# kkaytekin/Supervised-Depth-Estimation-from-Polarized-Images

Measured on AMD Instinct MI355X. Metric: train images/sec (512x612, 3-encoder), higher is better.
Workload: dtype f32; 1 GPU; BASELINE configs[2]: full 3-encoder (augment_xolp+augment_normals), multi-scale loss scales=[0,1,2,3], batch 16 per GPU, 512x612 frames (network/loss on 512x640 padded), dropout 0.1, Adam lr 1e-4, fp32; global_batch=16, height=512, width=640, frame_width=612, parallelism=dp1

## Files before the change

include/polardepth.h:

```cpp
#ifndef POLARDEPTH_H
#define POLARDEPTH_H

#include <stddef.h>
#include <stdint.h>

#ifdef __cplusplus
extern "C" {
#endif

#define PD_OK 0
#define PD_EINVAL (-22)
#define PD_ELAUNCH (-5)

const char* pd_last_error(void);
int pd_version(void);

#define PD_POLAR_LS 0
#define PD_POLAR_STOKES 1
#define PD_POLAR_PRECISE_NORMALS 1
#define PD_POLAR_IEEE_RHO 2
#define PD_POLAR_NT_LOADS 4
#define PD_POLAR_PLAIN_LOADS 8

size_t pd_polar_tables_bytes(int n_d, int n_s1, int n_s2);
// ... 12 lines not shown

int pd_polar_calc_normals(const void* phi, const void* theta, void* out, int B, long P, int phi_f64, int theta_f64,
                          void* stream);

int pd_polar_theta(const void* rho, void* theta_d, void* theta_s1, void* theta_s2, void* bins,
                   const void* tables, size_t tables_bytes, long n, void* stream);

#define PD_CONV_AUTO 0u
#define PD_CONV_FP32_MFMA 1u
#define PD_CONV_BF16X3 2u
#define PD_CONV_WGRAD_SPLIT_IN_REGS 4u
#define PD_CONV_GENERAL_KERNELS 8u
#define PD_CONV_X3_IM2COL 16u
#define PD_CONV_WGRAD_ROW_WORKGROUPS 32u
#define PD_CONV_BF16 128u
#define PD_CONV_FLAGS_ALL 191u
int pd_conv2d_tile_m(long M, int Cout);
long pd_conv2d_stats_rows(long M, int Cout);
int pd_conv2d_uses_x3(long M, int Cout, int C, int KH, int KW, int stride, int pad, int mode, int act, int has_out_scale,
                      int Ho, int Wo, unsigned flags);
int pd_conv2d_uses_bf16(long M, int Cout, int C, int KH, int KW, int stride, int pad, int mode, int act, int has_out_scale,
                        int Ho, int Wo, unsigned flags);
int pd_conv2d(const void* x, const void* w, const void* bias, const void* out_scale, void* y, void* stats,
              int N, int H, int W, int C, long sN, long sH, long sW, long sC,
              int Ho, int Wo, int Cout, int KH, int KW, int stride, int pad, int mode, int act,
              int affine, float sub, float div, long ldy, unsigned flags, void* stream);

int pd_conv16(const void* x, const void* w, const void* bias, void* y, int N, int H, int W, int C,
              long sN, long sH, long sW, int Ho, int Wo, int Cout, long ldy, int mode, int act, void* stream);

size_t pd_conv16_wgrad_workspace(int C);
int pd_conv16_wgrad(const void* x, const void* dz, void* dw, void* dbias, void* workspace, size_t ws_bytes,
                    int N, int H, int W, int C, long sN, long sH, long sW, long ldd, int accumulate, void* stream);

int pd_dgrad_s2_filters(const void* wt, void* wsub, int Cin, int Cout, void* stream);
int pd_conv2d_rect(const void* x, const void* w, void* y, int N, int H, int W, int C, long sN, long sH, long sW, long sC,
                   int Ho, int Wo, int Cout, int KH, int KW, int pad_h, int pad_w, int mode, long ldy, unsigned flags,
                   void* stream);
int pd_interleave4(const void* sub, void* dx, int N, int Ho, int Wo, int C, void* stream);

int pd_conv2d_add(const void* x, const void* w, const void* addend, long ld_add, void* y,
                  int N, int H, int W, int C, long sN, long sH, long sW, long sC,
                  int Ho, int Wo, int Cout, int KH, int KW, int stride, int pad, int mode, long ldy, unsigned flags,
                  void* stream);

size_t pd_conv2d_wgrad_workspace(long M, int Cout, int K, unsigned flags);
int pd_conv2d_wgrad(const void* x, const void* dy, void* dw, void* dbias, void* workspace, size_t ws_bytes,
                    int N, int H, int W, int C, long sN, long sH, long sW, long sC,
                    int Ho, int Wo, int Cout, int KH, int KW, int stride, int pad, int mode,
                    int affine, float sub, float div, long ldd, int accumulate, unsigned flags, void* stream);
int pd_conv2d_wgrad_uses_x3(long M, int Cout, int C, int KH, int KW, int stride, int pad, int mode, int H, int W, int Ho, int Wo,
                            unsigned flags);
int pd_conv2d_wgrad_uses_bf16(long M, int Cout, int C, int KH, int KW, int stride, int pad, int mode, int H, int W, int Ho, int Wo,
                              unsigned flags);

int pd_stem_s2d_input(const void* x, void* out, int N, int C, int H, int W, long sN, long sC, long sH, long sW,
                      int affine, float sub, float div, void* stream);
int pd_stem_s2d_weight(const void* w, void* w2, int Cout, int C, void* stream);
int pd_stem_s2d_weight_grad(const void* dw2, void* dw, int Cout, int C, int accumulate, void* stream);
// ... 131 lines not shown
```

supervised-depth-estimation-from-polarized-images_amd/csrc/conv.hip:

```cpp
#include "pd_common.h"
#include <cstdlib>
#include <type_traits>

namespace {

typedef float f32x16 __attribute__((ext_vector_type(16)));
typedef unsigned int u32x4 __attribute__((ext_vector_type(4)));

constexpr int BK = 32;
constexpr int LDT = BK;
constexpr int NT = 256;
constexpr unsigned OOB = 0x80000000u;

enum { MODE_ZERO = 0, MODE_REFLECT = 1, MODE_TRANSPOSED = 2 };
enum { ACT_NONE = 0, ACT_RELU = 1, ACT_ELU = 2, ACT_SIGMOID = 3 };

struct ConvArgs {
    const float* x;
    const float* w;
    const float* bias;
    const float* oscale;
    float* y;
    float* stats;
    const float* add;
// ... 4 lines not shown
    int KH, KW, stride, pad;
    int pad_w;
    int mode, act;
    int affine;
    float sub, div;
    int K;
    long M;
    long ldy;
    int mtiles, ntiles;
    int sshift;
    unsigned w_bytes;
    unsigned mg_hw, sh_hw, mg_wo, sh_wo;
    unsigned flags;
    int stats_rows;
    int nmajor;
};

__device__ __forceinline__ float4 ldg4(const float* p) { return *reinterpret_cast<const float4*>(p); }

__device__ __forceinline__ int swz(int row, int slot) { return 4 * (slot ^ ((row >> 1) & 7)); }

__device__ __forceinline__ __amdgpu_buffer_rsrc_t make_rsrc(const void* p, unsigned bytes) {
    return __builtin_amdgcn_make_buffer_rsrc(const_cast<void*>(p), 0, bytes, 0x00020000);
}
__device__ __forceinline__ float4 buf_ld4(__amdgpu_buffer_rsrc_t r, unsigned off) {
    return __builtin_bit_cast(float4, __builtin_amdgcn_raw_buffer_load_b128(r, off, 0, 0));
}
__device__ __forceinline__ float buf_ld1(__amdgpu_buffer_rsrc_t r, unsigned off) {
    return __builtin_bit_cast(float, __builtin_amdgcn_raw_buffer_load_b32(r, off, 0, 0));
}
// ... 637 lines not shown
template <int P, bool W = false> __device__ __forceinline__ void sp_m(const float* x, Terms& t) {
    if constexpr (PD_PROBE_RAW(W)) { t.m[P] = __float_as_uint(x[2 * P + 1]); return; }
    t.tf[P] = f32x2{__uint_as_float(t.h[P] << 16), __uint_as_float(t.h[P] & 0xffff0000u)};
    t.tr[P] = f32x2{x[2 * P], x[2 * P + 1]} - t.tf[P];
    t.m[P] = cvt_pk_bf16(t.tr[P].x, t.tr[P].y);
    t.tf[P].x = __uint_as_float(t.m[P] << 16);
}
template <int P, bool W = false> __device__ __forceinline__ void sp_l(Terms& t) {
    if constexpr (PD_PROBE_RAW(W)) { t.l[P] = t.h[P]; return; }
    t.tf[P].y = __uint_as_float(t.m[P] & 0xffff0000u);
    const f32x2 r2 = t.tr[P] - t.tf[P];
    t.l[P] = cvt_pk_bf16(r2.x, r2.y);
}
}

template <int MODE, int RB = 2>
__global__ __launch_bounds__(NT, RB == 2 ? 3 : 4) void conv_igemm_x3_kernel(const ConvArgs a) {
    using namespace x3;
    constexpr int BM = 128 * RB;
    constexpr unsigned A_BYTES = BM * CK * 4, BS_BASE = 2 * A_BYTES, BP_BASE = BS_BASE + 2 * BS_BYTES;
    constexpr unsigned LDS_BYTES = BP_BASE + 2 * 3 * BP_BYTES;
    __shared__ __attribute__((aligned(16))) float smem_all[LDS_BYTES / 4];

    const int nblk = a.mtiles * a.ntiles;
    const int per_xcd = (int)gridDim.x >> 3;
    const int logical = ((int)blockIdx.x & 7) * per_xcd + ((int)blockIdx.x >> 3);
    if (logical >= nblk) return;
    const int mt = a.nmajor ? logical % a.mtiles : logical / a.ntiles, nt = a.nmajor ? logical / a.mtiles : logical - mt * a.ntiles;
    const long m0 = (long)mt * BM;
    const int n0 = nt * BN;

    const int tid = threadIdx.x;
    const int lane = tid & 63;
    const int wave = __builtin_amdgcn_readfirstlane(tid >> 6);
    const int hw = a.Ho * a.Wo;

    const unsigned wsign = (mt & 1) ? 0x80008000u : 0u;
    const int img0 = (int)(m0 / hw);
    const long shift = MODE != MODE_TRANSPOSED ? (long)a.pad * a.sH + (long)a.pad_w * a.sW
                                               : (long)(a.KH - 1 - a.pad) * a.sH + (long)(a.KW - 1 - a.pad_w) * a.sW;
    const long rest = (((long)a.N - img0) * a.sN + shift) * 4;
    const __amdgpu_buffer_rsrc_t rx = make_rsrc(a.x + (long)img0 * a.sN - shift, rest > 0x7fffffffL ? 0x7fffffffu : (unsigned)rest);
    const __amdgpu_buffer_rsrc_t rw_ = make_rsrc(a.w, a.w_bytes);
// ... 27 lines not shown
            hi_w = ow + a.pad_w + 1; lo_w = hi_w - a.W;
        }
        lo_h = min(max(lo_h, 0), a.KH); hi_h = min(max(hi_h, 0), a.KH);
        lo_w = min(max(lo_w, 0), a.KW); hi_w = min(max(hi_w, 0), a.KW);
        const unsigned bad_h = ((1u << lo_h) - 1u) | ~((1u << hi_h) - 1u);
        const unsigned bad_w = (((1u << lo_w) - 1u) | ~((1u << hi_w) - 1u)) & ones_kw;
        unsigned mask = 0;
        for (int kh = a.KH - 1; kh >= 0; --kh)
            mask = (mask << a.KW) | (((bad_h >> kh) & 1u) ? ones_kw : bad_w);
        inv[i] = m < a.M ? (mask | 0x80000000u) : 0xffffffffu;
    }
    const unsigned vb = (unsigned)((n0 + 16 * wave + prow) * a.K) * 4u + col4;

    const int dW4 = (MODE != MODE_TRANSPOSED ? (int)a.sW : -(int)a.sW) * 4, dH4 = (MODE != MODE_TRANSPOSED ? (int)a.sH : -(int)a.sH) * 4;
    const int ngroups = (a.C + CK - 1) / CK;
    const int nchunks = ngroups * a.KH * a.KW;
    const int c_lim = a.C - 4 * ((lane & 3) ^ ((lane >> 4) & 3));
    const int ntaps = a.KH * a.KW;
    const unsigned aoff0 = MODE != MODE_TRANSPOSED ? 0u : (unsigned)(((a.KH - 1) * (int)a.sH + (a.KW - 1) * (int)a.sW) * 4);
    int s_q = 0, s_tap = 0, s_kw = 0, s_kh = 0, s_c = 0;
    unsigned s_aoff = aoff0;
    int s_qb = 0, sb_tap = 0;
    unsigned s_boff = 0, sb_c4 = 0;
    const unsigned lds0 = (unsigned)(size_t)(lds_ptr_t*)smem_all;
    const unsigned m0_a = lds0 + 2048u * RB * (unsigned)wave, m0_b = lds0 + BS_BASE + 1024u * (unsigned)wave;

    auto load_a = [&](auto dst_tag, auto piece_tag) {
        constexpr unsigned DST = decltype(dst_tag)::value;
        constexpr int P = decltype(piece_tag)::value;
        if constexpr (MODE == MODE_REFLECT) {
            const int hs = s_kh == 0 ? max(hcor[P], 0) : s_kh == 2 ? min(hcor[P], 0) : 0;
            const int ws = s_kw == 0 ? max(wcor[P], 0) : s_kw == 2 ? min(wcor[P], 0) : 0;
            const unsigned bad = (s_tap == 31 ? 1u : 0u) | ((unsigned)(c_lim - 1 - s_c) >> 31);
            dma16s(rx, m0_a + DST * A_BYTES + 1024u * P, (bad << 31) + (va[P] + (unsigned)(hs + ws)), s_aoff);
        } else {
        const unsigned bad = __builtin_amdgcn_ubfe(inv[P], (unsigned)s_tap, 1u) | ((unsigned)(c_lim - 1 - s_c) >> 31);
        dma16s(rx, m0_a + DST * A_BYTES + 1024u * P, (bad << 31) + va[P], s_aoff);
        }
// ... 138 lines not shown
        const std::integral_constant<unsigned, 1> d1{};
        pieces<0, 2 * RB>(load_a, d0);
        advance_a();
        load_b(d0);
        load_b(d1);
        asm volatile("s_waitcnt vmcnt(0)" ::: "memory");
        __syncthreads();
        split_b(d0);
        __syncthreads();
    }
    for (int q = 0; q < nchunks; q += 2) {
        chunk(std::integral_constant<unsigned, 0>{});
        if (q + 1 < nchunks) chunk(std::integral_constant<unsigned, 1>{});
    }

    {
        constexpr int RW = 32 * RB;
        float* T = smem_all + wave * (RW * 32);
        float (*red)[BN][2] = reinterpret_cast<float (*)[BN][2]>(smem_all + 4 * RW * 32);
        const int col_l = lane & 31, rbase = 4 * (lane >> 5);
        const bool elu = a.act == ACT_ELU;
        const long rows_here = a.M - m0 < BM ? a.M - m0 : BM;
        const __amdgpu_buffer_rsrc_t ry = make_rsrc(a.y + m0 * a.ldy, (unsigned)(rows_here * a.ldy * 4));
        const __amdgpu_buffer_rsrc_t ra = make_rsrc(a.add ? a.add + m0 * a.ld_add : a.y, a.add ? (unsigned)(rows_here * a.ld_add * 4) : 0u);
#pragma unroll
        for (int j = 0; j < 2; ++j) {
            float4 addv[4 * RB];
            if (a.add) {
                const unsigned off_a = (unsigned)((RW * wave + (lane >> 3)) * (int)a.ld_add + n0 + 32 * j + 4 * (lane & 7)) * 4u;
#pragma unroll
// ... 63 lines not shown
           (!a.add || ((a.ld_add & 3) == 0 && ((size_t)a.add & 15) == 0)) && (long)a.Co * a.K * 4 < 0x7fffffffL;
}
static int x3_eligible(const ConvArgs& a, bool vec) {
    const bool force = (a.flags & PD_CONV_BF16X3) != 0;
    if (!(x3_common_ok(a, vec) && (a.C + x3::CK - 1) / x3::CK * x3::CK <= 2 * a.C && a.Co % x3::BN == 0 &&
          (a.M % 128 == 0 || (a.mode == MODE_TRANSPOSED && !a.stats))))
        return 0;
    const long ct = a.Co / x3::BN;
    if (a.M % 256 == 0 && (a.M / 256) * ct >= X3_MIN_WG) return 2;
    return (force || (a.M / 128) * ct >= X3_MIN_WG1) ? 1 : 0;
}

static int x3_nmajor(const ConvArgs& a) { return (long)a.Co * a.K * 4 > (3L << 20) && a.ntiles >= 8 && a.ntiles % 8 == 0; }
#include "conv_x3_halo.hpp"

static int launch_conv_x3(ConvArgs& a, int rb, hipStream_t st) {
    a.mtiles = (int)((a.M + 128 * rb - 1) / (128 * rb));
    a.ntiles = a.Co / x3::BN;
    a.nmajor = x3_nmajor(a);
    const long nblk = (long)a.mtiles * a.ntiles;
    const dim3 grid((unsigned)((nblk + 7) / 8 * 8)), block(NT);
    if (rb == 2) {
        if (a.mode == MODE_ZERO) hipLaunchKernelGGL((conv_igemm_x3_kernel<MODE_ZERO, 2>), grid, block, 0, st, a);
        else if (a.mode == MODE_REFLECT) hipLaunchKernelGGL((conv_igemm_x3_kernel<MODE_REFLECT, 2>), grid, block, 0, st, a);
        else hipLaunchKernelGGL((conv_igemm_x3_kernel<MODE_TRANSPOSED, 2>), grid, block, 0, st, a);
    } else {
        if (a.mode == MODE_ZERO) hipLaunchKernelGGL((conv_igemm_x3_kernel<MODE_ZERO, 1>), grid, block, 0, st, a);
        else if (a.mode == MODE_REFLECT) hipLaunchKernelGGL((conv_igemm_x3_kernel<MODE_REFLECT, 1>), grid, block, 0, st, a);
        else hipLaunchKernelGGL((conv_igemm_x3_kernel<MODE_TRANSPOSED, 1>), grid, block, 0, st, a);
    }
    return pd::check_launch("pd_conv2d");
}

template <int BM, int BN, int WM, int WN>
int launch_conv(ConvArgs& a, bool vec, hipStream_t st) {
// ... 70 lines not shown

extern "C" int pd_conv2d_tile_m(long M, int Co) {
    if (Co <= 32) return 128;
    return M >= 64 * 1024 ? 128 : 64;
}

extern "C" long pd_conv2d_stats_rows(long M, int Co) {
    const int bm = pd_conv2d_tile_m(M, Co);
    return (M + bm - 1) / bm;
}

static int conv2d_impl(const void* x, const void* w, const void* bias, const void* out_scale, void* y, void* stats,
                       const void* addend, long ld_add,
                       int N, int H, int W, int C, long sN, long sH, long sW, long sC,
                       int Ho, int Wo, int Co, int KH, int KW, int stride, int pad, int mode, int act,
                       int affine, float sub, float div, long ldy, unsigned flags, void* stream, int pad_w = -1);

extern "C" int pd_conv2d(const void* x, const void* w, const void* bias, const void* out_scale, void* y, void* stats,
                         int N, int H, int W, int C, long sN, long sH, long sW, long sC,
                         int Ho, int Wo, int Co, int KH, int KW, int stride, int pad, int mode, int act,
                         int affine, float sub, float div, long ldy, unsigned flags, void* stream) {
    return conv2d_impl(x, w, bias, out_scale, y, stats, nullptr, 0, N, H, W, C, sN, sH, sW, sC, Ho, Wo, Co, KH, KW, stride,
                       pad, mode, act, affine, sub, div, ldy, flags, stream);
}

extern "C" int pd_conv2d_add(const void* x, const void* w, const void* addend, long ld_add, void* y,
                             int N, int H, int W, int C, long sN, long sH, long sW, long sC,
                             int Ho, int Wo, int Co, int KH, int KW, int stride, int pad, int mode, long ldy, unsigned flags,
                             void* stream) {
    PD_REQUIRE(addend && ld_add >= Co, "pd_conv2d_add: bad addend");
    return conv2d_impl(x, w, nullptr, nullptr, y, nullptr, addend, ld_add, N, H, W, C, sN, sH, sW, sC, Ho, Wo, Co, KH, KW,
                       stride, pad, mode, ACT_NONE, 0, 0.f, 1.f, ldy, flags, stream);
}

extern "C" int pd_conv2d_rect(const void* x, const void* w, void* y, int N, int H, int W, int C, long sN, long sH, long sW,
                              long sC, int Ho, int Wo, int Co, int KH, int KW, int pad_h, int pad_w, int mode, long ldy,
                              unsigned flags, void* stream) {
    PD_REQUIRE(pad_w >= 0 && mode != MODE_REFLECT, "pd_conv2d_rect: bad padding / mode");
    PD_REQUIRE(!(flags & PD_CONV_GENERAL_KERNELS), "pd_conv2d_rect: the general kernel has no separate column padding");
    return conv2d_impl(x, w, nullptr, nullptr, y, nullptr, nullptr, 0, N, H, W, C, sN, sH, sW, sC, Ho, Wo, Co, KH, KW, 1,
                       pad_h, mode, ACT_NONE, 0, 0.f, 1.f, ldy, flags, stream, pad_w);
}

static int conv2d_impl(const void* x, const void* w, const void* bias, const void* out_scale, void* y, void* stats,
                       const void* addend, long ld_add,
                       int N, int H, int W, int C, long sN, long sH, long sW, long sC,
                       int Ho, int Wo, int Co, int KH, int KW, int stride, int pad, int mode, int act,
                       int affine, float sub, float div, long ldy, unsigned flags, void* stream, int pad_w) {
    if (pad_w < 0) pad_w = pad;
    PD_REQUIRE(pd::conv_flags_ok(flags), "pd_conv2d: bad flags 0x%x", flags);
    PD_REQUIRE(x && w && y, "pd_conv2d: null tensor");
    PD_REQUIRE(N >= 0 && H > 0 && W > 0 && C > 0 && Ho > 0 && Wo > 0 && Co > 0, "pd_conv2d: bad dims");
    PD_REQUIRE(KH > 0 && KW > 0 && stride > 0 && pad >= 0, "pd_conv2d: bad filter geometry");
    PD_REQUIRE(mode >= 0 && mode <= 2 && act >= 0 && act <= 3, "pd_conv2d: bad mode/act");
    PD_REQUIRE(mode != MODE_REFLECT || (pad < H && pad < W), "pd_conv2d: reflect pad must be < input size");
    PD_REQUIRE(ldy >= Co && ldy < (1L << 22), "pd_conv2d: bad output row stride %ld (Cout=%d)", ldy, Co);
    int sshift = 0;
    while ((1 << sshift) < stride) ++sshift;
    if (mode == MODE_TRANSPOSED) {
        PD_REQUIRE((1 << sshift) == stride, "pd_conv2d: transposed mode needs a power-of-two stride");
        PD_REQUIRE(H <= (Ho + 2 * pad - KH) / stride + 1 && W <= (Wo + 2 * pad_w - KW) / stride + 1,
                   "pd_conv2d: transposed: x grid exceeds the forward output grid of a %dx%d input", Ho, Wo);
    } else {
        PD_REQUIRE(Ho <= (H + 2 * pad - KH) / stride + 1 && Wo <= (W + 2 * pad_w - KW) / stride + 1,
                   "pd_conv2d: output grid does not match input/filter geometry");
    }
    if (N == 0) return PD_OK;
    ConvArgs a;
    a.x = (const float*)x; a.w = (const float*)w; a.bias = (const float*)bias; a.oscale = (const float*)out_scale; a.y = (float*)y; a.stats = (float*)stats;
    a.add = (const float*)addend; a.ld_add = ld_add;
    a.N = N; a.H = H; a.W = W; a.C = C; a.sN = sN; a.sH = sH; a.sW = sW; a.sC = sC;
    a.Ho = Ho; a.Wo = Wo; a.Co = Co; a.KH = KH; a.KW = KW; a.stride = stride; a.pad = pad; a.pad_w = pad_w;
    a.mode = mode; a.act = act; a.affine = affine; a.sub = sub; a.div = div;
    a.K = KH * KW * C; a.M = (long)N * Ho * Wo; a.ldy = ldy; a.sshift = sshift;
    a.flags = flags; a.stats_rows = pd_conv2d_tile_m(a.M, Co);
    auto magic = [](long d, unsigned& mg, unsigned& sh) {
        if (d <= 1 || d >= (1L << 31)) { mg = 0; sh = 0; return; }
        int l = 0;
        while ((1L << l) < d) ++l;
        mg = (unsigned)((((unsigned long long)1 << (31 + l)) + (unsigned long long)d - 1) / (unsigned long long)d);
        sh = (unsigned)(l - 1);
    };
    magic((long)Ho * Wo, a.mg_hw, a.sh_hw);
    magic(Wo, a.mg_wo, a.sh_wo);
    const long wbytes = (long)Co * a.K * 4;
    PD_REQUIRE(wbytes < 0x7fffffffL, "pd_conv2d: weight tensor too large for 32-bit offsets");
    a.w_bytes = (unsigned)wbytes;
    const long span = 256 / ((long)Ho * Wo) + 2;
    PD_REQUIRE(span * sN * 4 < 0x7fffffffL, "pd_conv2d: image too large for 32-bit offsets (%ld bytes per image)", sN * 4);
    const bool vec = (C % 4 == 0) && sC == 1 && (sW % 4 == 0) && (sH % 4 == 0) && (sN % 4 == 0) && !affine &&
                     pd::aligned16(x) && pd::aligned16(w);
    hipStream_t st = (hipStream_t)stream;
    const int bm = pd_conv2d_tile_m(a.M, Co);
    if (x3_common_ok(a, vec) && !(flags & PD_CONV_X3_IM2COL) && x3_halo_eligible(a)) return launch_conv_x3_halo(a, st);
    if (const int rb = x3_eligible(a, vec)) return launch_conv_x3(a, rb, st);
    if (Co == 96 && bm == 128) return launch_conv<128, 32, 32, 32>(a, vec, st);
    if (Co > 32) return bm == 128 ? launch_conv<128, 64, 64, 32>(a, vec, st) : launch_conv<64, 64, 32, 32>(a, vec, st);
    if (Co > 16) return launch_conv<128, 32, 32, 32>(a, vec, st);
    return launch_conv<128, 16, 32, 16>(a, vec, st);
}

namespace {

constexpr int WG_K = 128;
constexpr int WG_MC = 32;
constexpr int WG_LDX = WG_K + 8;

struct WgradArgs {
    const float* x;
    const float* dy;
// ... 1249 lines not shown
```

supervised-depth-estimation-from-polarized-images_amd/polardepth/_lib.py:

```python
import ctypes
import os

_HERE = os.path.dirname(os.path.abspath(__file__))
_SO = os.environ.get("PD_LIB") or os.path.join(_HERE, "libpolardepth.so")


class LibraryMissing(RuntimeError):
    pass


class PolarDepthError(RuntimeError):
    pass


_c = ctypes
_vp, _i, _sz, _dbl = _c.c_void_p, _c.c_int, _c.c_size_t, _c.c_double
_dp = _c.POINTER(_c.c_double)
_l, _f = _c.c_long, _c.c_float
_u64 = _c.c_uint64
_ip = _c.POINTER(_c.c_int)
_u = _c.c_uint
_vpp = _c.POINTER(_c.c_void_p)

SIGNATURES = {
# ... 2 lines not shown
    "pd_polar_tables_bytes": (_sz, [_i, _i, _i]),
    "pd_polar_tables_pack": (_i, [_dp, _dp, _i, _dp, _dp, _i, _dp, _dp, _i, _vp, _sz]),
    "pd_polar_tables_build": (_i, [_dbl, _vp, _sz, _c.POINTER(_sz)]),
    "pd_polar_fwd": (_i, [_vp, _vp, _vp, _vp, _vp, _vp, _vp, _sz, _i, _i, _i, _i, _i, _i, _vp]),
    "pd_polar_normals_from_xolp": (_i, [_vp, _vp, _vp, _sz, _i, _i, _i, _i, _vp]),
    "pd_polar_theta": (_i, [_vp, _vp, _vp, _vp, _vp, _vp, _sz, _l, _vp]),
    "pd_polar_calc_normals": (_i, [_vp, _vp, _vp, _i, _l, _i, _i, _vp]),
    "pd_conv2d_tile_m": (_i, [_l, _i]),
    "pd_conv2d_stats_rows": (_l, [_l, _i]),
    "pd_conv2d_uses_x3": (_i, [_l, _i, _i, _i, _i, _i, _i, _i, _i, _i, _i, _i, _u]),
    "pd_conv2d_wgrad_uses_x3": (_i, [_l, _i, _i, _i, _i, _i, _i, _i, _i, _i, _i, _i, _u]),
    "pd_conv2d_uses_bf16": (_i, [_l, _i, _i, _i, _i, _i, _i, _i, _i, _i, _i, _i, _u]),
    "pd_conv2d_wgrad_uses_bf16": (_i, [_l, _i, _i, _i, _i, _i, _i, _i, _i, _i, _i, _i, _u]),
    "pd_conv2d": (_i, [_vp, _vp, _vp, _vp, _vp, _vp, _i, _i, _i, _i, _l, _l, _l, _l, _i, _i, _i, _i, _i, _i, _i, _i, _i,
                       _i, _f, _f, _l, _u, _vp]),
    "pd_conv16": (_i, [_vp, _vp, _vp, _vp, _i, _i, _i, _i, _l, _l, _l, _i, _i, _i, _l, _i, _i, _vp]),
    "pd_conv16_wgrad_workspace": (_sz, [_i]),
    "pd_conv16_wgrad": (_i, [_vp, _vp, _vp, _vp, _vp, _sz, _i, _i, _i, _i, _l, _l, _l, _l, _i, _vp]),
    "pd_dgrad_s2_filters": (_i, [_vp, _vp, _i, _i, _vp]),
    "pd_conv2d_rect": (_i, [_vp, _vp, _vp, _i, _i, _i, _i, _l, _l, _l, _l, _i, _i, _i, _i, _i, _i, _i, _i, _l, _u, _vp]),
    "pd_interleave4": (_i, [_vp, _vp, _i, _i, _i, _i, _vp]),
    "pd_conv2d_add": (_i, [_vp, _vp, _vp, _l, _vp, _i, _i, _i, _i, _l, _l, _l, _l, _i, _i, _i, _i, _i, _i, _i, _i, _l, _u, _vp]),
    "pd_conv2d_wgrad_workspace": (_sz, [_l, _i, _i, _u]),
    "pd_conv2d_wgrad": (_i, [_vp, _vp, _vp, _vp, _vp, _sz, _i, _i, _i, _i, _l, _l, _l, _l, _i, _i, _i, _i, _i, _i, _i,
                             _i, _i, _f, _f, _l, _i, _u, _vp]),
    "pd_weight_transpose": (_i, [_vp, _vp, _i, _i, _i, _vp]),
    "pd_weight_transpose_batched": (_i, [_vp, _vp, _vp, _vp, _i, _i, _vp]),
    "pd_stem_s2d_input": (_i, [_vp, _vp, _i, _i, _i, _i, _l, _l, _l, _l, _i, _f, _f, _vp]),
    "pd_stem_s2d_weight": (_i, [_vp, _vp, _i, _i, _vp]),
    "pd_stem_s2d_weight_grad": (_i, [_vp, _vp, _i, _i, _i, _vp]),
# ... 107 lines not shown
```

supervised-depth-estimation-from-polarized-images_amd/polardepth/ops.py:

```python
import os

import torch

from ._lib import lib, check, ptr, stream_ptr

MODE_ZERO, MODE_REFLECT, MODE_TRANSPOSED = 0, 1, 2
ACT_NONE, ACT_RELU, ACT_ELU, ACT_SIGMOID = 0, 1, 2, 3
CL = torch.channels_last
PROFILE = None

CONV_AUTO, CONV_FP32_MFMA, CONV_BF16X3, CONV_WGRAD_SPLIT_IN_REGS, CONV_GENERAL_KERNELS, CONV_X3_IM2COL = 0, 1, 2, 4, 8, 16
CONV_WGRAD_ROW_WORKGROUPS = 32
CONV_BF16 = 128
CONV_FLAGS = (CONV_FP32_MFMA if os.environ.get("PD_CONV_X3", "1") == "0" else
              CONV_X3_IM2COL if os.environ.get("PD_CONV_HALO", "1") == "0" else CONV_AUTO)
WGRAD_FLAGS = (CONV_FP32_MFMA if os.environ.get("PD_WGRAD_X3C", "1") == "0" else
               CONV_X3_IM2COL if os.environ.get("PD_CONV_HALO", "1") == "0" else
               CONV_WGRAD_ROW_WORKGROUPS if os.environ.get("PD_WGRAD_ROLL", "1") == "0" else CONV_AUTO)


class conv_flags:

    def __init__(self, conv=None, wgrad=None):
        self.new = (conv, wgrad)

    def __enter__(self):
        global CONV_FLAGS, WGRAD_FLAGS
        self.old = (CONV_FLAGS, WGRAD_FLAGS)
        if self.new[0] is not None:
            CONV_FLAGS = int(self.new[0])
# ... 63 lines not shown
def is_nhwc(t):
    n, c, h, w = t.shape
    return t.stride() == (h * w * c, 1, w * c, c) or t.is_contiguous(memory_format=CL)


def as_nhwc(t):
    return t if is_nhwc(t) else t.contiguous(memory_format=CL)


def weight_cl(w):
    return w if w.is_contiguous(memory_format=CL) else w.contiguous(memory_format=CL)


def conv_out_size(h, k, s, p):
    return (h + 2 * p - k) // s + 1


def conv2d_fwd(x, w, bias=None, stride=1, pad=0, mode=MODE_ZERO, act=ACT_NONE, want_stats=False,
               affine=None, out=None, out_hw=None, out_scale=None, alg_k=None):
    _require_cuda(x, w, bias, out_scale)
    global FWD_EPOCH
    FWD_EPOCH += 1
    N, C, H, W = x.shape
    Co, Ci, KH, KW = w.shape
    assert Ci == C, f"channel mismatch {Ci} vs {C}"
    w = weight_cl(w)
    Ho, Wo = conv_out_size(H, KH, stride, pad), conv_out_size(W, KW, stride, pad)
    if out_hw is not None:
        assert out_hw[0] <= Ho and out_hw[1] <= Wo
        Ho, Wo = out_hw
# ... 5 lines not shown
    stats = None
    if want_stats:
        rows = lib.pd_conv2d_stats_rows(N * Ho * Wo, Co)
        stats = torch.empty((rows, Co, 2), dtype=torch.float32, device=x.device)
    sub, div = (affine if affine is not None else (0.0, 1.0))
    sN, sC, sH, sW = x.stride()
    vec = C % 4 == 0 and sC == 1 and affine is None
    if (USE_CONV16 and mode == MODE_REFLECT and Co == 16 and C in (16, 32) and KH == 3 and KW == 3 and stride == 1 and pad == 1
            and vec and not want_stats and out_scale is None and act in (ACT_NONE, ACT_ELU) and out_hw is None
            and H >= 2 and W >= 2 and sN % 4 == 0 and sH % 4 == 0 and sW % 4 == 0):
        _profiled("conv16_halo_kernel", 2.0 * N * Ho * Wo * Co * C * 9,
                  lambda: check(lib.pd_conv16(ptr(x), ptr(w), ptr(bias), ptr(out), N, H, W, C, sN, sH, sW, Ho, Wo, Co, ldy,
                                              0, act, stream_ptr()), "pd_conv16"),
                  shape=("fwd", N, C, H, W, Co, KH, stride, mode))
        return out
    _profiled(_igemm_label(N * Ho * Wo, Co, vec, "fwd", C, KH, KW, stride, pad, mode, act, out_scale is not None, (Ho, Wo)), 2.0 * N * Ho * Wo * Co * (alg_k if alg_k is not None else C * KH * KW),
              lambda: check(lib.pd_conv2d(ptr(x), ptr(w), ptr(bias), ptr(out_scale), ptr(out), ptr(stats), N, H, W, C, sN, sH, sW, sC,
                                          Ho, Wo, Co, KH, KW, stride, pad, mode, act, int(affine is not None), sub,
                                          div, ldy, CONV_FLAGS, stream_ptr()), "pd_conv2d"),
              shape=("fwd", N, C, H, W, Co, KH, stride, mode))
    return (out, stats) if want_stats else out


USE_S2_PHASES = os.environ.get("PD_S2_PHASES", "1") != "0"
USE_CONV16 = os.environ.get("PD_CONV16", "1") != "0"
WT_PROVIDERS = []
FWD_EPOCH = 0


def weight_transposed(w):
    Co, Ci, KH, KW = w.shape
    w = weight_cl(w)
    for prov in WT_PROVIDERS:
        wt = prov.transposed(w)
# ... 26 lines not shown
                check(lib.pd_conv2d_rect(ptr(dy), wsub.data_ptr() + 4 * off * Ci * Co, ptr(sub[c]), N, Hy, Wy, Co, sN, sH, sW,
                                         sC, Hy, Wy, Ci, 1 + ph, 1 + pw, ph, pw, MODE_TRANSPOSED, Ci, flags, stream_ptr()),
                      "pd_conv2d_rect(dgrad s2 phase)")
            check(lib.pd_interleave4(ptr(sub), ptr(dx), N, Hy, Wy, Ci, stream_ptr()), "pd_interleave4")
        _profiled("conv_dgrad_s2_phases", 2.0 * N * Hy * Wy * Co * Ci * KH * KW, _phases,
                  shape=("dgrad", N, Ci, H, W, Co, KH, stride, MODE_TRANSPOSED))
        return dx
    c16_mode = 1 if (pad == 0 and H == Hy + 2 and W == Wy + 2) else (2 if (pad == 1 and H == Hy and W == Wy) else 0)
    if (USE_CONV16 and addend is None and Co == 16 and Ci in (16, 32) and KH == 3 and KW == 3 and stride == 1 and c16_mode
            and sC == 1 and sN % 4 == 0 and sH % 4 == 0 and sW % 4 == 0 and Hy >= 2 and Wy >= 2):
        _profiled("conv16_halo_kernel", 2.0 * N * Hy * Wy * Co * Ci * 9,
                  lambda: check(lib.pd_conv16(ptr(dy), ptr(wt), None, ptr(dx), N, Hy, Wy, Co, sN, sH, sW, H, W, Ci, Ci, c16_mode,
                                              0, stream_ptr()), "pd_conv16(dgrad)"),
                  shape=("dgrad", N, Ci, H, W, Co, KH, stride, MODE_TRANSPOSED))
        return dx
    if addend is not None:
        assert addend.shape == dx.shape and addend.stride(1) == 1 and addend.is_cuda
        ld_add = addend.stride(3)
        assert addend.stride(2) == W * ld_add and addend.stride(0) == H * W * ld_add
        _profiled(_igemm_label(N * H * W, Ci, True, "dgrad", Co, KH, KW, stride, pad, MODE_TRANSPOSED, out_hw=(H, W), flags=flags),
                  2.0 * N * Hy * Wy * Co * Ci * KH * KW,
                  lambda: check(lib.pd_conv2d_add(ptr(dy), ptr(wt), ptr(addend), ld_add, ptr(dx), N, Hy, Wy, Co, sN, sH, sW,
                                                  sC, H, W, Ci, KH, KW, stride, pad, MODE_TRANSPOSED, Ci, flags, stream_ptr()),
                                "pd_conv2d_add(dgrad)"),
                  shape=("dgrad", N, Ci, H, W, Co, KH, stride, MODE_TRANSPOSED))
        return dx
    _profiled(_igemm_label(N * H * W, Ci, True, "dgrad", Co, KH, KW, stride, pad, MODE_TRANSPOSED, out_hw=(H, W), flags=flags), 2.0 * N * Hy * Wy * Co * Ci * KH * KW,
              lambda: check(lib.pd_conv2d(ptr(dy), ptr(wt), None, None, ptr(dx), None, N, Hy, Wy, Co, sN, sH, sW, sC,
                                          H, W, Ci, KH, KW, stride, pad, MODE_TRANSPOSED, ACT_NONE, 0, 0.0, 1.0, Ci,
                                          flags, stream_ptr()), "pd_conv2d(dgrad)"),
              shape=("dgrad", N, Ci, H, W, Co, KH, stride, MODE_TRANSPOSED))
    return dx


_ws_cache = {}


def _workspace(nbytes, device):
    key = (device.index, torch.cuda.current_stream(device).cuda_stream)
    buf = _ws_cache.get(key)
    if buf is None or buf.numel() < nbytes:
        buf = torch.empty(max(nbytes, 1 << 20), dtype=torch.uint8, device=device)
        _ws_cache[key] = buf
    return buf

# ... 175 lines not shown
```

Measured before the change: 347.0 images/s.

## Add split-K to x3 implicit-GEMM conv for small-tile-count layers

Adds a split-K variant of the bf16x3 implicit-GEMM conv kernel. When a layer has few output tiles (at most 1280 workgroups after splitting) and enough channel groups, the K loop is divided into 2-4 slices. Each slice writes its partial tile to a workspace, and the last-arriving workgroup, chosen by an atomic ticket, sums the partials and runs the normal epilogue. The aim is to fill the GPU on deep, low-resolution encoder and decoder layers, for both forward and dgrad. The cost is extra global traffic for the partials, a cached zeroed workspace, and fence/atomic synchronisation.

```diff
diff --git a/include/polardepth.h b/include/polardepth.h
--- a/include/polardepth.h
+++ b/include/polardepth.h
@@ -50,7 +50,8 @@
 #define PD_CONV_X3_IM2COL 16u
 #define PD_CONV_WGRAD_ROW_WORKGROUPS 32u
 #define PD_CONV_BF16 128u
-#define PD_CONV_FLAGS_ALL 191u
+#define PD_CONV_NO_SPLITK 256u
+#define PD_CONV_FLAGS_ALL 447u
 int pd_conv2d_tile_m(long M, int Cout);
 long pd_conv2d_stats_rows(long M, int Cout);
 int pd_conv2d_uses_x3(long M, int Cout, int C, int KH, int KW, int stride, int pad, int mode, int act, int has_out_scale,
@@ -61,6 +62,13 @@
               int N, int H, int W, int C, long sN, long sH, long sW, long sC,
               int Ho, int Wo, int Cout, int KH, int KW, int stride, int pad, int mode, int act,
               int affine, float sub, float div, long ldy, unsigned flags, void* stream);
+size_t pd_conv2d_workspace(long M, int Cout, int C, int KH, int KW, int stride, int pad, int mode, int act, int has_out_scale,
+                           int Ho, int Wo, unsigned flags);
+int pd_conv2d_ws(const void* x, const void* w, const void* bias, const void* out_scale, void* y, void* stats,
+                 void* workspace, size_t ws_bytes,
+                 int N, int H, int W, int C, long sN, long sH, long sW, long sC,
+                 int Ho, int Wo, int Cout, int KH, int KW, int stride, int pad, int mode, int act,
+                 int affine, float sub, float div, long ldy, unsigned flags, void* stream);
 
 int pd_conv16(const void* x, const void* w, const void* bias, void* y, int N, int H, int W, int C,
               long sN, long sH, long sW, int Ho, int Wo, int Cout, long ldy, int mode, int act, void* stream);
@@ -79,6 +87,11 @@
                   int N, int H, int W, int C, long sN, long sH, long sW, long sC,
                   int Ho, int Wo, int Cout, int KH, int KW, int stride, int pad, int mode, long ldy, unsigned flags,
                   void* stream);
+int pd_conv2d_add_ws(const void* x, const void* w, const void* addend, long ld_add, void* y,
+                     void* workspace, size_t ws_bytes,
+                     int N, int H, int W, int C, long sN, long sH, long sW, long sC,
+                     int Ho, int Wo, int Cout, int KH, int KW, int stride, int pad, int mode, long ldy, unsigned flags,
+                     void* stream);
 
 size_t pd_conv2d_wgrad_workspace(long M, int Cout, int K, unsigned flags);
 int pd_conv2d_wgrad(const void* x, const void* dy, void* dw, void* dbias, void* workspace, size_t ws_bytes,
diff --git a/supervised-depth-estimation-from-polarized-images_amd/csrc/conv.hip b/supervised-depth-estimation-from-polarized-images_amd/csrc/conv.hip
--- a/supervised-depth-estimation-from-polarized-images_amd/csrc/conv.hip
+++ b/supervised-depth-estimation-from-polarized-images_amd/csrc/conv.hip
@@ -42,6 +42,9 @@
     unsigned flags;
     int stats_rows;
     int nmajor;
+    int splitk;
+    float* sk_part;
+    unsigned* sk_tickets;
 };
 
 __device__ __forceinline__ float4 ldg4(const float* p) { return *reinterpret_cast<const float4*>(p); }
@@ -709,8 +712,9 @@
 }
 }
 
-template <int MODE, int RB = 2>
+template <int MODE, int RB = 2, bool SK = false>
 __global__ __launch_bounds__(NT, RB == 2 ? 3 : 4) void conv_igemm_x3_kernel(const ConvArgs a) {
+    static_assert(!SK || RB == 1, "split-K: 128-row tiles only");
     using namespace x3;
     constexpr int BM = 128 * RB;
     constexpr unsigned A_BYTES = BM * CK * 4, BS_BASE = 2 * A_BYTES, BP_BASE = BS_BASE + 2 * BS_BYTES;
@@ -720,8 +724,9 @@
     const int nblk = a.mtiles * a.ntiles;
     const int per_xcd = (int)gridDim.x >> 3;
     const int logical = ((int)blockIdx.x & 7) * per_xcd + ((int)blockIdx.x >> 3);
-    if (logical >= nblk) return;
-    const int mt = a.nmajor ? logical % a.mtiles : logical / a.ntiles, nt = a.nmajor ? logical / a.mtiles : logical - mt * a.ntiles;
+    if (logical >= (SK ? nblk * a.splitk : nblk)) return;
+    const int tile = SK ? logical / a.splitk : logical, slice = SK ? logical - tile * a.splitk : 0;
+    const int mt = a.nmajor ? tile % a.mtiles : tile / a.ntiles, nt = a.nmajor ? tile / a.mtiles : tile - mt * a.ntiles;
     const long m0 = (long)mt * BM;
     const int n0 = nt * BN;
 
@@ -779,14 +784,15 @@
 
     const int dW4 = (MODE != MODE_TRANSPOSED ? (int)a.sW : -(int)a.sW) * 4, dH4 = (MODE != MODE_TRANSPOSED ? (int)a.sH : -(int)a.sH) * 4;
     const int ngroups = (a.C + CK - 1) / CK;
-    const int nchunks = ngroups * a.KH * a.KW;
+    const int g0 = SK ? slice * ngroups / a.splitk : 0, g1 = SK ? (slice + 1) * ngroups / a.splitk : ngroups;
+    const int nchunks = (g1 - g0) * a.KH * a.KW;
     const int c_lim = a.C - 4 * ((lane & 3) ^ ((lane >> 4) & 3));
     const int ntaps = a.KH * a.KW;
     const unsigned aoff0 = MODE != MODE_TRANSPOSED ? 0u : (unsigned)(((a.KH - 1) * (int)a.sH + (a.KW - 1) * (int)a.sW) * 4);
-    int s_q = 0, s_tap = 0, s_kw = 0, s_kh = 0, s_c = 0;
-    unsigned s_aoff = aoff0;
+    int s_q = 0, s_tap = 0, s_kw = 0, s_kh = 0, s_c = g0 * CK;
+    unsigned s_aoff = aoff0 + (unsigned)s_c * 4u;
     int s_qb = 0, sb_tap = 0;
-    unsigned s_boff = 0, sb_c4 = 0;
+    unsigned s_boff = (unsigned)g0 * (CK * 4), sb_c4 = s_boff;
     const unsigned lds0 = (unsigned)(size_t)(lds_ptr_t*)smem_all;
     const unsigned m0_a = lds0 + 2048u * RB * (unsigned)wave, m0_b = lds0 + BS_BASE + 1024u * (unsigned)wave;
 
@@ -955,6 +961,53 @@
         if (q + 1 < nchunks) chunk(std::integral_constant<unsigned, 1>{});
     }
 
+    if constexpr (SK) {
+        const int S = a.splitk;
+        float4* part = reinterpret_cast<float4*>(a.sk_part) + (long)tile * S * (BM * BN / 4) + tid;
+        float4* mine = part + slice * (BM * BN / 4);
+#pragma unroll
+        for (int j = 0; j < 2; ++j)
+#pragma unroll
+            for (int q = 0; q < 4; ++q)
+                mine[(4 * j + q) * NT] = float4{acc[0][j][4 * q], acc[0][j][4 * q + 1], acc[0][j][4 * q + 2], acc[0][j][4 * q + 3]};
+        asm volatile("s_waitcnt vmcnt(0)" ::: "memory");
+        __syncthreads();
+        unsigned* last_s = reinterpret_cast<unsigned*>(smem_all);
+        if (tid == 0) {
+            __builtin_amdgcn_fence(__ATOMIC_RELEASE, "agent");
+            asm volatile("s_waitcnt vmcnt(0)" ::: "memory");
+            *last_s = __hip_atomic_fetch_add(a.sk_tickets + tile, 1u, __ATOMIC_RELAXED, __HIP_MEMORY_SCOPE_AGENT);
+        }
+        __syncthreads();
+        if (*last_s != (unsigned)(S - 1)) return;
+        if (tid == 0) {
+            __builtin_amdgcn_fence(__ATOMIC_ACQUIRE, "agent");
+            asm volatile("s_waitcnt vmcnt(0)" ::: "memory");
+            __hip_atomic_store(a.sk_tickets + tile, 0u, __ATOMIC_RELAXED, __HIP_MEMORY_SCOPE_AGENT);
+        }
+        __syncthreads();
+        {
+            float4 v[8];
+#pragma unroll
+            for (int e = 0; e < 8; ++e) v[e] = part[e * NT];
+#pragma unroll
+            for (int e = 0; e < 8; ++e) {
+                const int j = e >> 2, q = e & 3;
+                acc[0][j][4 * q] = v[e].x; acc[0][j][4 * q + 1] = v[e].y; acc[0][j][4 * q + 2] = v[e].z; acc[0][j][4 * q + 3] = v[e].w;
+            }
+        }
+        for (int s = 1; s < S; ++s) {
+            float4 v[8];
+#pragma unroll
+            for (int e = 0; e < 8; ++e) v[e] = part[s * (BM * BN / 4) + e * NT];
+#pragma unroll
+            for (int e = 0; e < 8; ++e) {
+                const int j = e >> 2, q = e & 3;
+                acc[0][j][4 * q] += v[e].x; acc[0][j][4 * q + 1] += v[e].y; acc[0][j][4 * q + 2] += v[e].z; acc[0][j][4 * q + 3] += v[e].w;
+            }
+        }
+    }
+
     {
         constexpr int RW = 32 * RB;
         float* T = smem_all + wave * (RW * 32);
@@ -1048,11 +1101,42 @@
 static int x3_nmajor(const ConvArgs& a) { return (long)a.Co * a.K * 4 > (3L << 20) && a.ntiles >= 8 && a.ntiles % 8 == 0; }
 #include "conv_x3_halo.hpp"
 
-static int launch_conv_x3(ConvArgs& a, int rb, hipStream_t st) {
+constexpr long X3_SK_MAX_WG = 1280;
+constexpr size_t X3_SK_TICKET_BYTES = 64 << 10;
+constexpr size_t X3_SK_SLICE_BYTES = 128 * x3::BN * 4;
+static int x3_splitk(long tiles, int groups, unsigned flags) {
+    if (flags & PD_CONV_NO_SPLITK) return 1;
+#ifdef PD_X3_SPLITK_FORCE
+    return tiles * PD_X3_SPLITK_FORCE <= 4 * X3_SK_MAX_WG && groups >= 2 * PD_X3_SPLITK_FORCE ? PD_X3_SPLITK_FORCE : 1;
+#endif
+    for (int s = 4; s >= 2; --s)
+        if (tiles * s <= X3_SK_MAX_WG && groups >= 2 * s) return s;
+    return 1;
+}
+static int x3_splitk(const ConvArgs& a) {
+    return x3_splitk((a.M + 127) / 128 * (a.Co / x3::BN), (a.C + x3::CK - 1) / x3::CK, a.flags);
+}
+static size_t x3_splitk_bytes(long tiles, int S) { return X3_SK_TICKET_BYTES + (size_t)tiles * S * X3_SK_SLICE_BYTES; }
+
+static int launch_conv_x3(ConvArgs& a, int rb, hipStream_t st, void* workspace = nullptr, size_t ws_bytes = 0) {
     a.mtiles = (int)((a.M + 128 * rb - 1) / (128 * rb));
     a.ntiles = a.Co / x3::BN;
     a.nmajor = x3_nmajor(a);
     const long nblk = (long)a.mtiles * a.ntiles;
+    const int S = rb == 1 && workspace ? x3_splitk(a) : 1;
+    if (S > 1) {
+        PD_REQUIRE(ws_bytes >= x3_splitk_bytes(nblk, S) && ((size_t)workspace & 15) == 0,
+                   "pd_conv2d: split-K workspace too small or misaligned (%zu bytes, pd_conv2d_workspace: %zu)", ws_bytes,
+                   x3_splitk_bytes(nblk, S));
+        a.splitk = S;
+        a.sk_tickets = static_cast<unsigned*>(workspace);
+        a.sk_part = reinterpret_cast<float*>(static_cast<char*>(workspace) + X3_SK_TICKET_BYTES);
+        const dim3 grid((unsigned)((nblk * S + 7) / 8 * 8)), block(NT);
+        if (a.mode == MODE_ZERO) hipLaunchKernelGGL((conv_igemm_x3_kernel<MODE_ZERO, 1, true>), grid, block, 0, st, a);
+        else if (a.mode == MODE_REFLECT) hipLaunchKernelGGL((conv_igemm_x3_kernel<MODE_REFLECT, 1, true>), grid, block, 0, st, a);
+        else hipLaunchKernelGGL((conv_igemm_x3_kernel<MODE_TRANSPOSED, 1, true>), grid, block, 0, st, a);
+        return pd::check_launch("pd_conv2d");
+    }
     const dim3 grid((unsigned)((nblk + 7) / 8 * 8)), block(NT);
     if (rb == 2) {
         if (a.mode == MODE_ZERO) hipLaunchKernelGGL((conv_igemm_x3_kernel<MODE_ZERO, 2>), grid, block, 0, st, a);
@@ -1153,7 +1237,8 @@
                        const void* addend, long ld_add,
                        int N, int H, int W, int C, long sN, long sH, long sW, long sC,
                        int Ho, int Wo, int Co, int KH, int KW, int stride, int pad, int mode, int act,
-                       int affine, float sub, float div, long ldy, unsigned flags, void* stream, int pad_w = -1);
+                       int affine, float sub, float div, long ldy, unsigned flags, void* stream, int pad_w = -1,
+                       void* workspace = nullptr, size_t ws_bytes = 0);
 
 extern "C" int pd_conv2d(const void* x, const void* w, const void* bias, const void* out_scale, void* y, void* stats,
                          int N, int H, int W, int C, long sN, long sH, long sW, long sC,
@@ -1172,6 +1257,34 @@
                        stride, pad, mode, ACT_NONE, 0, 0.f, 1.f, ldy, flags, stream);
 }
 
+extern "C" size_t pd_conv2d_workspace(long M, int Co, int C, int KH, int KW, int stride, int pad, int mode, int act,
+                                      int has_out_scale, int Ho, int Wo, unsigned flags) {
+    if (!pd::conv_flags_ok(flags) || pd_conv2d_uses_x3(M, Co, C, KH, KW, stride, pad, mode, act, has_out_scale, Ho, Wo, flags) != 1)
+        return 0;
+    const long tiles = (M + 127) / 128 * (Co / x3::BN);
+    const int S = x3_splitk(tiles, (C + x3::CK - 1) / x3::CK, flags);
+    return S > 1 ? x3_splitk_bytes(tiles, S) : 0;
+}
+
+extern "C" int pd_conv2d_ws(const void* x, const void* w, const void* bias, const void* out_scale, void* y, void* stats,
+                            void* workspace, size_t ws_bytes,
+                            int N, int H, int W, int C, long sN, long sH, long sW, long sC,
+                            int Ho, int Wo, int Co, int KH, int KW, int stride, int pad, int mode, int act,
+                            int affine, float sub, float div, long ldy, unsigned flags, void* stream) {
+    return conv2d_impl(x, w, bias, out_scale, y, stats, nullptr, 0, N, H, W, C, sN, sH, sW, sC, Ho, Wo, Co, KH, KW, stride,
+                       pad, mode, act, affine, sub, div, ldy, flags, stream, -1, workspace, ws_bytes);
+}
+
+extern "C" int pd_conv2d_add_ws(const void* x, const void* w, const void* addend, long ld_add, void* y,
+                                void* workspace, size_t ws_bytes,
+                                int N, int H, int W, int C, long sN, long sH, long sW, long sC,
+                                int Ho, int Wo, int Co, int KH, int KW, int stride, int pad, int mode, long ldy, unsigned flags,
+                                void* stream) {
+    PD_REQUIRE(addend && ld_add >= Co, "pd_conv2d_add: bad addend");
+    return conv2d_impl(x, w, nullptr, nullptr, y, nullptr, addend, ld_add, N, H, W, C, sN, sH, sW, sC, Ho, Wo, Co, KH, KW,
+                       stride, pad, mode, ACT_NONE, 0, 0.f, 1.f, ldy, flags, stream, -1, workspace, ws_bytes);
+}
+
 extern "C" int pd_conv2d_rect(const void* x, const void* w, void* y, int N, int H, int W, int C, long sN, long sH, long sW,
                               long sC, int Ho, int Wo, int Co, int KH, int KW, int pad_h, int pad_w, int mode, long ldy,
                               unsigned flags, void* stream) {
@@ -1185,7 +1298,8 @@
                        const void* addend, long ld_add,
                        int N, int H, int W, int C, long sN, long sH, long sW, long sC,
                        int Ho, int Wo, int Co, int KH, int KW, int stride, int pad, int mode, int act,
-                       int affine, float sub, float div, long ldy, unsigned flags, void* stream, int pad_w) {
+                       int affine, float sub, float div, long ldy, unsigned flags, void* stream, int pad_w,
+                       void* workspace, size_t ws_bytes) {
     if (pad_w < 0) pad_w = pad;
     PD_REQUIRE(pd::conv_flags_ok(flags), "pd_conv2d: bad flags 0x%x", flags);
     PD_REQUIRE(x && w && y, "pd_conv2d: null tensor");
@@ -1206,6 +1320,7 @@
     }
     if (N == 0) return PD_OK;
     ConvArgs a;
+    a.splitk = 1; a.sk_part = nullptr; a.sk_tickets = nullptr;
     a.x = (const float*)x; a.w = (const float*)w; a.bias = (const float*)bias; a.oscale = (const float*)out_scale; a.y = (float*)y; a.stats = (float*)stats;
     a.add = (const float*)addend; a.ld_add = ld_add;
     a.N = N; a.H = H; a.W = W; a.C = C; a.sN = sN; a.sH = sH; a.sW = sW; a.sC = sC;
@@ -1232,7 +1347,7 @@
     hipStream_t st = (hipStream_t)stream;
     const int bm = pd_conv2d_tile_m(a.M, Co);
     if (x3_common_ok(a, vec) && !(flags & PD_CONV_X3_IM2COL) && x3_halo_eligible(a)) return launch_conv_x3_halo(a, st);
-    if (const int rb = x3_eligible(a, vec)) return launch_conv_x3(a, rb, st);
+    if (const int rb = x3_eligible(a, vec)) return launch_conv_x3(a, rb, st, workspace, ws_bytes);
     if (Co == 96 && bm == 128) return launch_conv<128, 32, 32, 32>(a, vec, st);
     if (Co > 32) return bm == 128 ? launch_conv<128, 64, 64, 32>(a, vec, st) : launch_conv<64, 64, 32, 32>(a, vec, st);
     if (Co > 16) return launch_conv<128, 32, 32, 32>(a, vec, st);
diff --git a/supervised-depth-estimation-from-polarized-images_amd/polardepth/_lib.py b/supervised-depth-estimation-from-polarized-images_amd/polardepth/_lib.py
--- a/supervised-depth-estimation-from-polarized-images_amd/polardepth/_lib.py
+++ b/supervised-depth-estimation-from-polarized-images_amd/polardepth/_lib.py
@@ -40,6 +40,11 @@
     "pd_conv2d_wgrad_uses_bf16": (_i, [_l, _i, _i, _i, _i, _i, _i, _i, _i, _i, _i, _i, _u]),
     "pd_conv2d": (_i, [_vp, _vp, _vp, _vp, _vp, _vp, _i, _i, _i, _i, _l, _l, _l, _l, _i, _i, _i, _i, _i, _i, _i, _i, _i,
                        _i, _f, _f, _l, _u, _vp]),
+    "pd_conv2d_workspace": (_sz, [_l, _i, _i, _i, _i, _i, _i, _i, _i, _i, _i, _i, _u]),
+    "pd_conv2d_ws": (_i, [_vp, _vp, _vp, _vp, _vp, _vp, _vp, _sz, _i, _i, _i, _i, _l, _l, _l, _l, _i, _i, _i, _i, _i, _i, _i, _i,
+                          _i, _i, _f, _f, _l, _u, _vp]),
+    "pd_conv2d_add_ws": (_i, [_vp, _vp, _vp, _l, _vp, _vp, _sz, _i, _i, _i, _i, _l, _l, _l, _l, _i, _i, _i, _i, _i, _i, _i, _i, _l,
+                              _u, _vp]),
     "pd_conv16": (_i, [_vp, _vp, _vp, _vp, _i, _i, _i, _i, _l, _l, _l, _i, _i, _i, _l, _i, _i, _vp]),
     "pd_conv16_wgrad_workspace": (_sz, [_i]),
     "pd_conv16_wgrad": (_i, [_vp, _vp, _vp, _vp, _vp, _sz, _i, _i, _i, _i, _l, _l, _l, _l, _i, _vp]),
diff --git a/supervised-depth-estimation-from-polarized-images_amd/polardepth/ops.py b/supervised-depth-estimation-from-polarized-images_amd/polardepth/ops.py
--- a/supervised-depth-estimation-from-polarized-images_amd/polardepth/ops.py
+++ b/supervised-depth-estimation-from-polarized-images_amd/polardepth/ops.py
@@ -12,8 +12,11 @@
 CONV_AUTO, CONV_FP32_MFMA, CONV_BF16X3, CONV_WGRAD_SPLIT_IN_REGS, CONV_GENERAL_KERNELS, CONV_X3_IM2COL = 0, 1, 2, 4, 8, 16
 CONV_WGRAD_ROW_WORKGROUPS = 32
 CONV_BF16 = 128
+CONV_NO_SPLITK = 256
 CONV_FLAGS = (CONV_FP32_MFMA if os.environ.get("PD_CONV_X3", "1") == "0" else
               CONV_X3_IM2COL if os.environ.get("PD_CONV_HALO", "1") == "0" else CONV_AUTO)
+if os.environ.get("PD_CONV_SPLITK", "1") == "0":
+    CONV_FLAGS |= CONV_NO_SPLITK
 WGRAD_FLAGS = (CONV_FP32_MFMA if os.environ.get("PD_WGRAD_X3C", "1") == "0" else
                CONV_X3_IM2COL if os.environ.get("PD_CONV_HALO", "1") == "0" else
                CONV_WGRAD_ROW_WORKGROUPS if os.environ.get("PD_WGRAD_ROLL", "1") == "0" else CONV_AUTO)
@@ -107,6 +110,31 @@
 
 def conv_out_size(h, k, s, p):
     return (h + 2 * p - k) // s + 1
+
+
+SPLITK_TICKET_BYTES = 64 << 10
+SPLITK_BYTES = SPLITK_TICKET_BYTES + 1280 * 128 * 64 * 4
+_sk_cache = {}
+_sk_retired = []
+
+
+def _splitk_workspace(nbytes, device):
+    if not nbytes:
+        return None
+    key = (device.index, torch.cuda.current_stream(device).cuda_stream)
+    buf = _sk_cache.get(key)
+    if buf is None or buf.numel() < nbytes:
+        if buf is not None:
+            _sk_retired.append(buf)
+        buf = torch.zeros(max(nbytes, SPLITK_BYTES), dtype=torch.uint8, device=device)
+        _sk_cache[key] = buf
+    return buf
+
+
+def _check_splitk(rc, what, sk):
+    if rc != 0 and sk is not None:
+        sk[:SPLITK_TICKET_BYTES].zero_()
+    check(rc, what)
 
 
 def conv2d_fwd(x, w, bias=None, stride=1, pad=0, mode=MODE_ZERO, act=ACT_NONE, want_stats=False,
@@ -142,10 +170,13 @@
                                               0, act, stream_ptr()), "pd_conv16"),
                   shape=("fwd", N, C, H, W, Co, KH, stride, mode))
         return out
+    sk = _splitk_workspace(lib.pd_conv2d_workspace(N * Ho * Wo, Co, C, KH, KW, stride, pad, mode, act, int(out_scale is not None),
+                                                   Ho, Wo, CONV_FLAGS) if vec else 0, x.device)
     _profiled(_igemm_label(N * Ho * Wo, Co, vec, "fwd", C, KH, KW, stride, pad, mode, act, out_scale is not None, (Ho, Wo)), 2.0 * N * Ho * Wo * Co * (alg_k if alg_k is not None else C * KH * KW),
-              lambda: check(lib.pd_conv2d(ptr(x), ptr(w), ptr(bias), ptr(out_scale), ptr(out), ptr(stats), N, H, W, C, sN, sH, sW, sC,
-                                          Ho, Wo, Co, KH, KW, stride, pad, mode, act, int(affine is not None), sub,
-                                          div, ldy, CONV_FLAGS, stream_ptr()), "pd_conv2d"),
+              lambda: _check_splitk(lib.pd_conv2d_ws(ptr(x), ptr(w), ptr(bias), ptr(out_scale), ptr(out), ptr(stats), ptr(sk),
+                                                     sk.numel() if sk is not None else 0, N, H, W, C, sN, sH, sW, sC,
+                                                     Ho, Wo, Co, KH, KW, stride, pad, mode, act, int(affine is not None), sub,
+                                                     div, ldy, CONV_FLAGS, stream_ptr()), "pd_conv2d", sk),
               shape=("fwd", N, C, H, W, Co, KH, stride, mode))
     return (out, stats) if want_stats else out
 
@@ -202,21 +233,24 @@
                                               0, stream_ptr()), "pd_conv16(dgrad)"),
                   shape=("dgrad", N, Ci, H, W, Co, KH, stride, MODE_TRANSPOSED))
         return dx
+    sk = _splitk_workspace(lib.pd_conv2d_workspace(N * H * W, Ci, Co, KH, KW, stride, pad, MODE_TRANSPOSED, ACT_NONE, 0, H, W, flags),
+                           dy.device)
+    nsk = sk.numel() if sk is not None else 0
     if addend is not None:
         assert addend.shape == dx.shape and addend.stride(1) == 1 and addend.is_cuda
         ld_add = addend.stride(3)
         assert addend.stride(2) == W * ld_add and addend.stride(0) == H * W * ld_add
         _profiled(_igemm_label(N * H * W, Ci, True, "dgrad", Co, KH, KW, stride, pad, MODE_TRANSPOSED, out_hw=(H, W), flags=flags),
                   2.0 * N * Hy * Wy * Co * Ci * KH * KW,
-                  lambda: check(lib.pd_conv2d_add(ptr(dy), ptr(wt), ptr(addend), ld_add, ptr(dx), N, Hy, Wy, Co, sN, sH, sW,
-                                                  sC, H, W, Ci, KH, KW, stride, pad, MODE_TRANSPOSED, Ci, flags, stream_ptr()),
-                                "pd_conv2d_add(dgrad)"),
+                  lambda: _check_splitk(lib.pd_conv2d_add_ws(ptr(dy), ptr(wt), ptr(addend), ld_add, ptr(dx), ptr(sk), nsk, N, Hy, Wy,
+                                                             Co, sN, sH, sW, sC, H, W, Ci, KH, KW, stride, pad, MODE_TRANSPOSED, Ci,
+                                                             flags, stream_ptr()), "pd_conv2d_add(dgrad)", sk),
                   shape=("dgrad", N, Ci, H, W, Co, KH, stride, MODE_TRANSPOSED))
         return dx
     _profiled(_igemm_label(N * H * W, Ci, True, "dgrad", Co, KH, KW, stride, pad, MODE_TRANSPOSED, out_hw=(H, W), flags=flags), 2.0 * N * Hy * Wy * Co * Ci * KH * KW,
-              lambda: check(lib.pd_conv2d(ptr(dy), ptr(wt), None, None, ptr(dx), None, N, Hy, Wy, Co, sN, sH, sW, sC,
-                                          H, W, Ci, KH, KW, stride, pad, MODE_TRANSPOSED, ACT_NONE, 0, 0.0, 1.0, Ci,
-                                          flags, stream_ptr()), "pd_conv2d(dgrad)"),
+              lambda: _check_splitk(lib.pd_conv2d_ws(ptr(dy), ptr(wt), None, None, ptr(dx), None, ptr(sk), nsk, N, Hy, Wy, Co,
+                                                     sN, sH, sW, sC, H, W, Ci, KH, KW, stride, pad, MODE_TRANSPOSED, ACT_NONE, 0,
+                                                     0.0, 1.0, Ci, flags, stream_ptr()), "pd_conv2d(dgrad)", sk),
               shape=("dgrad", N, Ci, H, W, Co, KH, stride, MODE_TRANSPOSED))
     return dx
 
```

Result: no change. 346.6 images/s (-0.1%).
